# Chthi/Ofighters

Measured on AMD Instinct MI355X. Metric: arena-steps/sec (env.step+obs+policy fwd) at 4096 arenas, 1/2/4/8 MI355X, higher is better.
Workload: dtype f32; 1 GPU; 4096 arenas x 8 ships per GPU, random-bot actions + step + 2D obs rasterise (u8 maps) + bi-head policy forward for 8 ship(s)/arena, trunk shared per arena (BASELINE configs[3]); arenas_per_gpu=4096, ships=8, laser_cap=512, episode_ticks=200, parallelism=arena-sharded x1, RCCL all-reduce of episodic scores only, laser_overflow=0, last_episode_score_sum=70993, last_episode_arenas=4096

## Files before the change

### ofighters_amd/csrc/ofx_trunk.hip

```cpp
#include "ofx_trunk.h"
#include "ofx_diag.h"
#include "ofx_lowp.h"

typedef float f32x4 __attribute__((ext_vector_type(4)));
typedef float f32x2 __attribute__((ext_vector_type(2)));

template <int CIN, int COUT, int TH, int TW, int MODE, bool POOL, bool OUT_HWC>
__global__ __launch_bounds__(((TH / 2) * (TW / 2) + 63) / 64 * 64) void k_conv(ConvParams p) {
  constexpr int NT = (TH / 2) * (TW / 2);
  constexpr int NTB = (NT + 63) / 64 * 64;
  constexpr int TWP = TW + 2;
  __shared__ __align__(16) float tile[CIN][TH + 2][TWP];
  const int img = blockIdx.x / p.tiles, t = blockIdx.x - img * p.tiles;
  if (p.mask && !p.mask[img]) return;
  const int ty0 = (t / p.tiles_x) * TH, tx0 = (t % p.tiles_x) * TW;
  const int tid = threadIdx.x;
  const int H = p.H, W = p.W;

  constexpr int TOTAL = CIN * (TH + 2) * TWP;
  constexpr int SU = 8;
  for (int base = 0; base < TOTAL; base += NTB * SU) {
    float vals[SU];
#pragma unroll
    for (int u = 0; u < SU; u++) {
      const int e = base + u * NTB + tid;
      float v = 0.f;
      if (e < TOTAL) {
        const int c = e % TWP, r = (e / TWP) % (TH + 2), ci = e / (TWP * (TH + 2));
        const int gy = ty0 - 1 + r, gx = tx0 - 1 + c;
        if (gy >= 0 && gy < H && gx >= 0 && gx < W) {
          if (MODE == 0) {
            v = p.in[(((size_t)img * CIN + ci) * H + gy) * W + gx];
          } else if (MODE == 1) {
            const int cell = gy * W + gx;
            v = (float)((p.bits[ci][(size_t)img * p.bits_stride + (cell >> 5)] >> (cell & 31)) & 1u);
          }
        }
      }
      vals[u] = v;
    }
#pragma unroll
    for (int u = 0; u < SU; u++) {
      const int e = base + u * NTB + tid;
      if (e < TOTAL) (&tile[0][0][0])[e] = vals[u];
    }
  }
  __syncthreads();
  if (tid >= NT) return;
  const int tr = tid / (TW / 2), tc = tid - tr * (TW / 2);

  float acc[2][2][COUT];
#pragma unroll
  for (int i = 0; i < 2; i++)
#pragma unroll
    for (int j = 0; j < 2; j++)
#pragma unroll
      for (int co = 0; co < COUT; co++) acc[i][j][co] = 0.f;

#pragma unroll
  for (int ci = 0; ci < CIN; ci++) {
    float v[4][4];
#pragma unroll
    for (int r = 0; r < 4; r++) {
      const float2 lo = *reinterpret_cast<const float2 *>(&tile[ci][2 * tr + r][2 * tc]);
      const float2 hi = *reinterpret_cast<const float2 *>(&tile[ci][2 * tr + r][2 * tc + 2]);
      v[r][0] = lo.x; v[r][1] = lo.y; v[r][2] = hi.x; v[r][3] = hi.y;
    }
#pragma unroll
    for (int dy = 0; dy < 3; dy++)
#pragma unroll
      for (int dx = 0; dx < 3; dx++)
#pragma unroll
        for (int co = 0; co < COUT; co++) {
          const float wv = p.w[((dy * 3 + dx) * CIN + ci) * COUT + co];
#pragma unroll
          for (int i = 0; i < 2; i++)
#pragma unroll
            for (int j = 0; j < 2; j++) acc[i][j][co] = __builtin_fmaf(v[i + dy][j + dx], wv, acc[i][j][co]);
        }
  }

  const int oy = ty0 + 2 * tr, ox = tx0 + 2 * tc;
#pragma unroll
  for (int co = 0; co < COUT; co++) {
    const float bias = p.b[co];
// ... 218 lines not shown
  p.H = H; p.W = H;
  p.tiles_x = (H + 16 * NG - 1) / (16 * NG);
  p.tiles = p.tiles_x * (H / TH);
  if (p.tiles % TPW) { ofx_set_error("launch_convm: %d tiles per image not divisible by %d", p.tiles, TPW); return OFX_ERR_INVALID; }
  if (OUT_HWC && (H % 2 || H > 16 * NG)) { ofx_set_error("launch_convm: the 8-byte staging takes even rows of one tile width"); return OFX_ERR_INVALID; }
  p.images = images;
  hipLaunchKernelGGL((k_convm<CIN, TH, NG, MODE, OUT_HWC, TPW, LP>), dim3((unsigned)((images + 7) / 8 * 8 * (p.tiles / TPW))), dim3(256), 0,
                     h->stream, p);
  OFX_HIP(hipGetLastError());
  return OFX_OK;
}

template <int TH>
__global__ __launch_bounds__(256) void k_conv1_lut(ConvParams p, const float *lut) {
  constexpr int W = PS, H = PS, WR = 14;
  constexpr int W2 = W / 2, NPX = (TH / 2) * W2;
  __shared__ __align__(16) float slut[2 * 512 * 8];
  __shared__ unsigned rows[2][TH + 2][WR];
  const int tiles = H / TH;
  const int img = blockIdx.x / tiles, ty0 = (blockIdx.x - img * tiles) * TH;
  const int tid = threadIdx.x;
  for (int e = tid; e < 2 * 512 * 8 / 4; e += 256)
    reinterpret_cast<float4 *>(slut)[e] = reinterpret_cast<const float4 *>(lut)[e];
  for (int e = tid; e < 2 * (TH + 2) * WR; e += 256) {
    const int w = e % WR, r = (e / WR) % (TH + 2), ci = e / (WR * (TH + 2));
    const int gy = ty0 - 1 + r;
    unsigned out = 0u;
    if (gy >= 0 && gy < H) {
      const long long s0 = (long long)gy * W + 32 * w - 1;
      const unsigned *bits = p.bits[ci] + (size_t)img * p.bits_stride;
      const long long sw = s0 >> 5;
      const unsigned lo = (sw >= 0 && sw < (PS * PS) >> 5) ? bits[sw] : 0u;
      const unsigned hi = (sw + 1 < (PS * PS) >> 5) ? bits[sw + 1] : 0u;
      out = __funnelshift_r(lo, hi, (unsigned)(s0 & 31));
      const int xlo = 32 * w - 1;
      if (xlo < 0) out &= ~1u;
      const int over = xlo + 32 - W;
      if (over > 0) out = over >= 32 ? 0u : (out & (0xFFFFFFFFu >> over));
    }
    rows[ci][r][w] = out;
  }
  __syncthreads();
  float *const obase = p.out + ((size_t)img * 8 * (H / 2) + (ty0 >> 1)) * W2;
  constexpr int NQ = NPX / 4, QR = W2 / 4;
  for (int qd = tid; qd < NQ; qd += 256) {
    const int py = qd / QR, pq = qd - py * QR;
    const int x0 = 8 * pq;
    unsigned f[2][4];
#pragma unroll
    for (int ci = 0; ci < 2; ci++)
#pragma unroll
      for (int r = 0; r < 4; r++) {
        const unsigned *rw = &rows[ci][2 * py + r][x0 >> 5];
        f[ci][r] = __funnelshift_r(rw[0], rw[1], (unsigned)(x0 & 31)) & 1023u;
      }
    f32x4 m4[8];
#pragma unroll
    for (int j = 0; j < 4; j++) {
      f32x4 acc[4][2];
#pragma unroll
      for (int ci = 0; ci < 2; ci++)
#pragma unroll
        for (int q = 0; q < 4; q++) {
          const int dy = q >> 1, sh = 2 * j + (q & 1);
          const unsigned pat = ((f[ci][dy] >> sh) & 7u) | (((f[ci][dy + 1] >> sh) & 7u) << 3) | (((f[ci][dy + 2] >> sh) & 7u) << 6);
          const f32x4 *e = reinterpret_cast<const f32x4 *>(&slut[(ci * 512 + pat) * 8]);
          if (ci == 0) { acc[q][0] = e[0]; acc[q][1] = e[1]; }
          else { acc[q][0] += e[0]; acc[q][1] += e[1]; }
        }
#pragma unroll
      for (int co = 0; co < 8; co++) {
        float m;
        asm("v_max3_f32 %0, %1, %2, 0" : "=v"(m) : "v"(acc[0][co >> 2][co & 3]), "v"(acc[1][co >> 2][co & 3]));
        asm("v_max3_f32 %0, %1, %2, %3" : "=v"(m) : "v"(acc[2][co >> 2][co & 3]), "v"(acc[3][co >> 2][co & 3]), "v"(m));
        m4[co][j] = m;
      }
    }
    const unsigned off = (unsigned)(py * W2 + 4 * pq);
#pragma unroll
    for (int co = 0; co < 8; co++) *reinterpret_cast<f32x4 *>(obase + (size_t)co * (H / 2) * W2 + off) = m4[co];
  }
}

template <int WD, int RP, int LS, int PLS>
__device__ __forceinline__ void ts_gemm_phase(const float *abase, const float (&bw)[24], const f32x4 binit, int wv, int n16,
                                              int kq, int r, float *orow) {
  constexpr int NK = 24, NPX = RP * WD, NT = (NPX + 15) / 16;
  static_assert(WD % 4 == 0 && NT <= 64, "four M-tiles per wave at most");
  auto aof = [&](int j) -> int { return (4 * (j & 1)) * PLS + ((j >> 1) / 3) * LS + ((j >> 1) % 3); };
  auto finish = [&](const f32x4 d, int T) {
    float q0, q1;
    q0 = max_raw(max_raw(d[0], 0.f), d[1]);
    q1 = max_raw(max_raw(d[2], 0.f), d[3]);
    q0 = max_raw(q0, __builtin_bit_cast(float, __builtin_amdgcn_mov_dpp(__builtin_bit_cast(int, q0), 0xB1, 0xF, 0xF, true)));
    q1 = max_raw(q1, __builtin_bit_cast(float, __builtin_amdgcn_mov_dpp(__builtin_bit_cast(int, q1), 0xB1, 0xF, 0xF, true)));
    const int P = 16 * T + 4 * kq;
    const int rp = P / WD, x = P - rp * WD;
    if (r == 0 && P < NPX) *reinterpret_cast<float2 *>(orow + rp * (WD / 2) + (x >> 1)) = make_float2(q0, q1);
  };
  auto a_of_tile = [&](int T) -> const float * {
    const int P = min(16 * T + n16, NPX - 1);
    const int rp = P / WD, x = P - rp * WD;
    return abase + 2 * rp * LS + x;
  };
  if (wv + 48 < NT) {
    const float *a0 = a_of_tile(wv), *a1 = a_of_tile(wv + 16), *a2 = a_of_tile(wv + 32), *a3 = a_of_tile(wv + 48);
    f32x4 d0 = binit, d1 = binit, d2 = binit, d3 = binit;
#pragma unroll
    for (int j = 0; j < NK; j++) {
      d0 = __builtin_amdgcn_mfma_f32_16x16x4f32(a0[aof(j)], bw[j], d0, 0, 0, 0);
      d1 = __builtin_amdgcn_mfma_f32_16x16x4f32(a1[aof(j)], bw[j], d1, 0, 0, 0);
      d2 = __builtin_amdgcn_mfma_f32_16x16x4f32(a2[aof(j)], bw[j], d2, 0, 0, 0);
      d3 = __builtin_amdgcn_mfma_f32_16x16x4f32(a3[aof(j)], bw[j], d3, 0, 0, 0);
    }
    finish(d0, wv); finish(d1, wv + 16); finish(d2, wv + 32); finish(d3, wv + 48);
  } else {
#pragma unroll 1
    for (int T = wv; T < NT; T += 32) {
      const int T1 = T + 16;
      const float *a0 = a_of_tile(T);
      if (T1 < NT) {
        const float *a1 = a_of_tile(T1);
        f32x4 d0 = binit, d1 = binit;
#pragma unroll
        for (int j = 0; j < NK; j++) {
          d0 = __builtin_amdgcn_mfma_f32_16x16x4f32(a0[aof(j)], bw[j], d0, 0, 0, 0);
          d1 = __builtin_amdgcn_mfma_f32_16x16x4f32(a1[aof(j)], bw[j], d1, 0, 0, 0);
        }
        finish(d0, T);
        finish(d1, T1);
      } else {
        f32x4 d0 = binit;
#pragma unroll
        for (int j = 0; j < NK; j++) d0 = __builtin_amdgcn_mfma_f32_16x16x4f32(a0[aof(j)], bw[j], d0, 0, 0, 0);
        finish(d0, T);
      }
    }
  }
}

template <int WD, int RP, int LS, int PLS, int LP>
__device__ __forceinline__ void ts_gemm_phase_sparse(const float *abase, const float (&bw)[LP ? 1 : 24], const lp_x4 (&bwb)[6],
                                                     const f32x4 binit, int wv, int lane,
                                                     int n16, int kq, int r, float *orow, const unsigned *nz, float k2,
                                                     bool top, bool bottom, unsigned &n_exec, unsigned &n_all,
                                                     unsigned long long *dbg = nullptr) {
#if OFX_TRUNK_STAMPS
  unsigned long long g_last = __builtin_amdgcn_s_memtime();
#define TSG_STAMP(i) do { const unsigned long long t_ = __builtin_amdgcn_s_memtime(); dbg[i] += t_ - g_last; g_last = t_; } while (0)
#else
#define TSG_STAMP(i) do { } while (0)
#endif
  constexpr int NK = 24, NPX = RP * WD, NT = (NPX + 15) / 16;
  static_assert(WD % 4 == 0 && NT <= 64, "four M-tiles per wave at most");
  auto aof = [&](int j) -> int { return (4 * (j & 1)) * PLS + ((j >> 1) / 3) * LS + ((j >> 1) % 3); };
  int toff[6];
#pragma unroll
  for (int J = 0; J < 6; J++) {
    const int tap = 2 * J + (kq >> 1);
    toff[J] = (4 * (kq & 1) - kq) * PLS + (tap / 3) * LS + tap % 3;
  }
  auto mm1 = [&](const float *a0, f32x4 &d0) {
    if constexpr (LP != 0) {
#pragma unroll
      for (int J = 0; J < 6; J++) {
        const float *q0 = a0 + toff[J];
        d0 = lp_mfma16<LP ? LP : 1>(lp_pk4<LP ? LP : 1>(q0[0], q0[PLS], q0[2 * PLS], q0[3 * PLS]), bwb[J], d0);
      }
    } else {
#pragma unroll
      for (int j = 0; j < NK; j++) d0 = __builtin_amdgcn_mfma_f32_16x16x4f32(a0[aof(j)], bw[LP ? 0 : j], d0, 0, 0, 0);
    }
  };
  auto mm2 = [&](const float *a0, const float *a1, f32x4 &d0, f32x4 &d1) {
    if constexpr (LP != 0) {
#pragma unroll
      for (int J = 0; J < 6; J++) {
        const float *q0 = a0 + toff[J], *q1 = a1 + toff[J];
        const lp_x4 A0 = lp_pk4<LP ? LP : 1>(q0[0], q0[PLS], q0[2 * PLS], q0[3 * PLS]);
        const lp_x4 A1 = lp_pk4<LP ? LP : 1>(q1[0], q1[PLS], q1[2 * PLS], q1[3 * PLS]);
        d0 = lp_mfma16<LP ? LP : 1>(A0, bwb[J], d0);
        d1 = lp_mfma16<LP ? LP : 1>(A1, bwb[J], d1);
      }
    } else {
#pragma unroll
      for (int j = 0; j < NK; j++) {
        d0 = __builtin_amdgcn_mfma_f32_16x16x4f32(a0[aof(j)], bw[LP ? 0 : j], d0, 0, 0, 0);
        d1 = __builtin_amdgcn_mfma_f32_16x16x4f32(a1[aof(j)], bw[LP ? 0 : j], d1, 0, 0, 0);
      }
    }
  };
  auto finish = [&](const f32x4 d, int T) {
    float q0, q1;
    q0 = max_raw(max_raw(d[0], 0.f), d[1]);
    q1 = max_raw(max_raw(d[2], 0.f), d[3]);
    q0 = max_raw(q0, __builtin_bit_cast(float, __builtin_amdgcn_mov_dpp(__builtin_bit_cast(int, q0), 0xB1, 0xF, 0xF, true)));
    q1 = max_raw(q1, __builtin_bit_cast(float, __builtin_amdgcn_mov_dpp(__builtin_bit_cast(int, q1), 0xB1, 0xF, 0xF, true)));
    const int P = 16 * T + 4 * kq;
    const int rp = P / WD, x = P - rp * WD;
    if (r == 0 && P < NPX) *reinterpret_cast<float2 *>(orow + rp * (WD / 2) + (x >> 1)) = make_float2(q0, q1);
  };
  auto a_of_tile = [&](int T) -> const float * {
    const int P = min(16 * T + n16, NPX - 1);
    const int rp = P / WD, x = P - rp * WD;
    return abase + 2 * rp * LS + x;
  };
  unsigned long long run_mask;
  {
    const int T = lane, P = 16 * T, rp = P / WD, x = P - rp * WD;
    bool run = T < NT;
    if (run && !(x < 1 || x + 15 > WD - 2 || P + 15 >= NPX || (top && rp == 0) || (bottom && rp == RP - 1))) {
      const int w0 = (x - 1) >> 5, lo = (x - 1) & 31;
      const unsigned m0 = 0x3FFFFu << lo, m1 = lo + 18 > 32 ? (1u << (lo + 18 - 32)) - 1u : 0u;
      unsigned any = 0u;
#pragma unroll
      for (int rr = 0; rr < 4; rr++) {
        const unsigned *rw = nz + (2 * rp + rr) * 8 + w0;
        any |= (rw[0] & m0) | (rw[1] & m1);
      }
      run = any != 0u;
    }
    run_mask = __builtin_amdgcn_ballot_w64(run);
  }
  auto store_const = [&](int T) {
    const int P = 16 * T + 4 * kq, rp = P / WD, x = P - rp * WD;
    if (r == 0) *reinterpret_cast<float2 *>(orow + rp * (WD / 2) + (x >> 1)) = make_float2(k2, k2);
  };
  auto run1 = [&](int T0) {
    f32x4 d0 = binit;
    mm1(a_of_tile(T0), d0);
    finish(d0, T0);
  };
#pragma unroll 1
  for (int T = wv; T < NT; T += 16)
    if (!((run_mask >> T) & 1ull)) store_const(T);
  if (wv == 0) { n_all += (unsigned)NT; n_exec += (unsigned)__builtin_popcountll(run_mask); }
  TSG_STAMP(0);
  unsigned long long m = run_mask;
  for (int i = 0; i < wv && m; i++) m &= m - 1;
#pragma unroll 1
  while (m) {
    const int T0 = __builtin_ctzll(m);
    unsigned long long m2 = m;
    for (int i = 0; i < 16 && m2; i++) m2 &= m2 - 1;
    if (m2) {
      const int T1 = __builtin_ctzll(m2);
      f32x4 d0 = binit, d1 = binit;
      mm2(a_of_tile(T0), a_of_tile(T1), d0, d1);
      finish(d0, T0);
      finish(d1, T1);
      for (int i = 0; i < 16 && m2; i++) m2 &= m2 - 1;
    } else run1(T0);
    m = m2;
  }
  TSG_STAMP(2);
}

template <int WD, int RP, int LS, int PLS, int LP>
__device__ __forceinline__ void ts_gemm_phase_bf16(const float *abase, const lp_x4 (&bwb)[6], const f32x4 binit, int wv, int n16,
                                                   int kq, int r, float *orow) {
  constexpr int NPX = RP * WD, NT = (NPX + 15) / 16;
  static_assert(WD % 4 == 0 && NT <= 64, "four M-tiles per wave at most");
  int toff[6];
#pragma unroll
  for (int J = 0; J < 6; J++) {
    const int tap = 2 * J + (kq >> 1);
    toff[J] = (4 * (kq & 1) - kq) * PLS + (tap / 3) * LS + tap % 3;
  }
  auto finish = [&](const f32x4 d, int T) {
    float q0, q1;
    q0 = max_raw(max_raw(d[0], 0.f), d[1]);
    q1 = max_raw(max_raw(d[2], 0.f), d[3]);
    q0 = max_raw(q0, __builtin_bit_cast(float, __builtin_amdgcn_mov_dpp(__builtin_bit_cast(int, q0), 0xB1, 0xF, 0xF, true)));
    q1 = max_raw(q1, __builtin_bit_cast(float, __builtin_amdgcn_mov_dpp(__builtin_bit_cast(int, q1), 0xB1, 0xF, 0xF, true)));
    const int P = 16 * T + 4 * kq;
    const int rp = P / WD, x = P - rp * WD;
    if (r == 0 && P < NPX) *reinterpret_cast<float2 *>(orow + rp * (WD / 2) + (x >> 1)) = make_float2(q0, q1);
  };
  auto a_of_tile = [&](int T) -> const float * {
    const int P = min(16 * T + n16, NPX - 1);
    const int rp = P / WD, x = P - rp * WD;
    return abase + 2 * rp * LS + x;
  };
#pragma unroll 1
  for (int T = wv; T < NT; T += 32) {
    const int T1 = T + 16;
    const bool two = T1 < NT;
    const float *a0 = a_of_tile(T), *a1 = a_of_tile(two ? T1 : T);
    f32x4 d0 = binit, d1 = binit;
#pragma unroll
    for (int J = 0; J < 6; J++) {
      const float *q0 = a0 + toff[J], *q1 = a1 + toff[J];
      const lp_x4 A0 = lp_pk4<LP>(q0[0], q0[PLS], q0[2 * PLS], q0[3 * PLS]);
      const lp_x4 A1 = lp_pk4<LP>(q1[0], q1[PLS], q1[2 * PLS], q1[3 * PLS]);
      d0 = lp_mfma16<LP>(A0, bwb[J], d0);
      d1 = lp_mfma16<LP>(A1, bwb[J], d1);
    }
    finish(d0, T);
    if (two) finish(d1, T1);
  }
}

constexpr int F12_TH = 10, F12_LS = 216, F12_ROWS = F12_TH + 2;
constexpr int F12_PLS = (F12_ROWS * F12_LS + 63) / 64 * 64 + 16;
constexpr int F12_WR = 14, F12_BR = 2 * (F12_TH + 1) + 2;
constexpr int F12_THREADS = 1024;
static_assert(F12_PLS % 64 == 16 && F12_PLS % 4 == 0 && F12_LS % 4 == 0, "tile layout");
static_assert(2 * F12_BR * F12_WR <= F12_THREADS, "one staged word per thread");
static_assert((F12_TH + 1) * 100 <= 2 * F12_THREADS && F12_TH * 100 <= F12_THREADS, "pixel pairs per step");

template <int LP, bool SPARSE = false>
__global__ __launch_bounds__(F12_THREADS) void k_trunk12(ConvParams p, const float *lut) {
  constexpr bool BF16 = LP != 0;
  constexpr int W = PS, H = PS, H1 = PS / 2, H2 = PS / 4, LS = F12_LS, PLS = F12_PLS, NK = 24;
  __shared__ __align__(16) float slut[2 * 512 * 8];
  __shared__ __align__(16) float tile[8 * F12_PLS];
  __shared__ unsigned rows[2][2][F12_BR][F12_WR];
  __shared__ __align__(16) float halo[2][8][2][F12_LS];
  __shared__ unsigned nz[SPARSE ? 2 : 1][F12_ROWS][8];
  __shared__ __align__(16) float k1s[8], k2s[8];
  __shared__ float wbs[(SPARSE && !BF16) ? 24 * 64 : 1];
  unsigned n_exec = 0, n_all = 0, t_exec = 0, t_all = 0;
#if OFX_TRUNK_STAMPS
  unsigned long long st_a = 0, st_b = 0, st_last = __builtin_amdgcn_s_memtime(), st_begin = st_last, st_g[3] = {0, 0, 0};
#define T12_STAMP(acc) do { const unsigned long long t_ = __builtin_amdgcn_s_memtime(); acc += t_ - st_last; st_last = t_; } while (0)
#else
#define T12_STAMP(acc) do { } while (0)
#endif
  const int tid = threadIdx.x, lane = tid & 63;
  const int wv = __builtin_amdgcn_readfirstlane(tid >> 6);
  const int n16 = lane & 15, kq = lane >> 4, co = n16 >> 1, r = n16 & 1;

  auto bits_fetch = [&](int img, int pa, int pb) -> unsigned {
    const int nrows = 2 * (pb - pa) + 2;
    unsigned out = 0u;
    if (tid < 2 * nrows * F12_WR) {
      const int w = tid % F12_WR, rr = (tid / F12_WR) % nrows, ci = tid / (F12_WR * nrows);
      const int gy = 2 * pa - 1 + rr;
      if (gy >= 0 && gy < H) {
        const long long s0 = (long long)gy * W + 32 * w - 1;
        const unsigned *bits = p.bits[ci] + (size_t)img * p.bits_stride;
        const long long sw = s0 >> 5;
        const unsigned lo = (sw >= 0 && sw < (PS * PS) >> 5) ? bits[sw] : 0u;
        const unsigned hi = (sw + 1 < (PS * PS) >> 5) ? bits[sw + 1] : 0u;
        out = __funnelshift_r(lo, hi, (unsigned)(s0 & 31));
        const int xlo = 32 * w - 1;
        if (xlo < 0) out &= ~1u;
        const int over = xlo + 32 - W;
        if (over > 0) out = over >= 32 ? 0u : (out & (0xFFFFFFFFu >> over));
      }
    }
    return out;
  };
  auto bits_commit = [&](int buf, int pa, int pb, unsigned word) {
    const int nrows = 2 * (pb - pa) + 2;
    if (tid < 2 * nrows * F12_WR) {
      const int w = tid % F12_WR, rr = (tid / F12_WR) % nrows, ci = tid / (F12_WR * nrows);
      rows[buf][ci][rr][w] = word;
    }
  };

  for (int e = tid; e < 2 * 512 * 8 / 4; e += F12_THREADS)
    reinterpret_cast<f32x4 *>(slut)[e] = reinterpret_cast<const f32x4 *>(lut)[e];
  for (int e = tid; e < 8 * PLS / 4; e += F12_THREADS) reinterpret_cast<f32x4 *>(tile)[e] = f32x4{0.f, 0.f, 0.f, 0.f};
  for (int e = tid; e < 2 * 8 * 2 * LS / 4; e += F12_THREADS) reinterpret_cast<f32x4 *>(&halo[0][0][0][0])[e] = f32x4{0.f, 0.f, 0.f, 0.f};
  float bw[(BF16 || SPARSE) ? 1 : NK];
  lp_x4 bwb[6];
  if constexpr (BF16) ts_bw_lp<LP ? LP : 1>(p.wbm, n16, kq, bwb);
  else if constexpr (SPARSE) {
    for (int e = tid; e < NK * 64; e += F12_THREADS) wbs[e] = p.wbm[e];
  } else {
#pragma unroll
    for (int j = 0; j < NK; j++) bw[j] = p.wbm[j * 64 + lane];
  }
  const float bias = p.b[co];
  const f32x4 binit = {bias, bias, bias, bias};
  const float *abase = &tile[kq * PLS + 3];
  if constexpr (SPARSE) {
    __syncthreads();
    if (tid < 8) k1s[tid] = fmaxf(slut[tid] + slut[512 * 8 + tid], 0.f);
    for (int e = tid; e < 2 * F12_ROWS * 8; e += F12_THREADS) (&nz[0][0][0])[e] = 0u;
    __syncthreads();
    for (int e = tid; e < 8 * PLS; e += F12_THREADS) tile[e] = k1s[min(e / PLS, 7)];
    __syncthreads();
    if (wv == 0) {
      const float *a0 = abase + 2 * LS + 16 + n16;
      f32x4 d0 = binit;
      if constexpr (BF16) {
#pragma unroll
        for (int J = 0; J < 6; J++) {
          const int tap = 2 * J + (kq >> 1);
          const float *q0 = a0 + (4 * (kq & 1) - kq) * PLS + (tap / 3) * LS + tap % 3;
          d0 = lp_mfma16<LP ? LP : 1>(lp_pk4<LP ? LP : 1>(q0[0], q0[PLS], q0[2 * PLS], q0[3 * PLS]), bwb[J], d0);
        }
      } else {
        auto aof = [&](int j) -> int { return (4 * (j & 1)) * PLS + ((j >> 1) / 3) * LS + ((j >> 1) % 3); };
#pragma unroll
        for (int j = 0; j < NK; j++) d0 = __builtin_amdgcn_mfma_f32_16x16x4f32(a0[aof(j)], wbs[(BF16 ? 0 : j) * 64 + lane], d0, 0, 0, 0);
      }
      float q0 = max_raw(max_raw(d0[0], 0.f), d0[1]);
      q0 = max_raw(q0, __builtin_bit_cast(float, __builtin_amdgcn_mov_dpp(__builtin_bit_cast(int, q0), 0xB1, 0xF, 0xF, true)));
      if (r == 0 && kq == 0) k2s[co] = q0;
    }
    __syncthreads();
    for (int e = tid; e < 8 * PLS / 4; e += F12_THREADS) reinterpret_cast<f32x4 *>(tile)[e] = f32x4{0.f, 0.f, 0.f, 0.f};
  }
  bits_commit(0, 0, F12_TH + 1, bits_fetch((int)blockIdx.x, 0, F12_TH + 1));
  unsigned w_ahead = 0u;
  if constexpr (SPARSE) { if ((int)blockIdx.x < p.images) w_ahead = bits_fetch((int)blockIdx.x, F12_TH + 1, 2 * F12_TH + 1); }
  __syncthreads();
  const float k2 = SPARSE ? k2s[co] : 0.f;

#pragma unroll 1
  for (int img = (int)blockIdx.x; img < p.images; img += (int)gridDim.x)
#pragma unroll 1
  for (int step = 0; step < H1 / F12_TH; step++) {
    const int R0 = step * F12_TH;
    const int pa = step ? R0 + 1 : 0, pb = min(R0 + F12_TH + 1, H1);
    const int buf = step & 1;
    const bool last = step + 1 == H1 / F12_TH;
    const int nimg = last ? img + (int)gridDim.x : img;
    const bool more = nimg < p.images;
    const int na = last ? 0 : R0 + F12_TH + 1, nb = last ? F12_TH + 1 : min(R0 + 2 * F12_TH + 1, H1);
    unsigned nextw = 0u;
    T12_STAMP(st_b);
    if (step && pb - pa < F12_TH)
      for (int e = tid; e < 8 * LS; e += F12_THREADS) tile[(e / LS) * PLS + (F12_TH + 1) * LS + e % LS] = 0.f;
    if (!step)
      for (int e = tid; e < 8 * LS; e += F12_THREADS) tile[(e / LS) * PLS + e % LS] = 0.f;
    if (step && tid < 8 * 2 * (LS / 4)) {
      const int c4 = tid % (LS / 4), rr = (tid / (LS / 4)) & 1, ci = tid / (2 * (LS / 4));
      reinterpret_cast<f32x4 *>(&tile[ci * PLS + rr * LS])[c4] = reinterpret_cast<const f32x4 *>(&halo[buf][ci][rr][0])[c4];
    }
    if constexpr (SPARSE) {
      if (step && tid < 16) nz[buf][tid >> 3][tid & 7] = nz[buf ^ 1][F12_TH + (tid >> 3)][tid & 7];
    }
    for (int q = tid; q < (pb - pa) * 100; q += F12_THREADS) {
      const int py = q / 100, pp = q - py * 100;
      const int x0 = 4 * pp;
      unsigned f[2][4];
#pragma unroll
      for (int ci = 0; ci < 2; ci++)
#pragma unroll
        for (int rr = 0; rr < 4; rr++) {
          const unsigned *rw = &rows[buf][ci][2 * py + rr][x0 >> 5];
          f[ci][rr] = __funnelshift_r(rw[0], rw[1], (unsigned)(x0 & 31)) & 63u;
        }
      float m2[8][2];
      bool dense_pass = true;
      if constexpr (SPARSE) {
        const unsigned any = (f[0][0] | f[0][1] | f[0][2] | f[0][3]) | (f[1][0] | f[1][1] | f[1][2] | f[1][3]);
        dense_pass = __builtin_amdgcn_ballot_w64(any != 0u) != 0;
        t_all++;
        if (dense_pass) {
          t_exec++;
          if (any != 0u) atomicOr(&nz[buf][pa + py - (R0 - 1)][(2 * pp) >> 5], 3u << ((2 * pp) & 31));
        } else {
          const f32x4 ka = *reinterpret_cast<const f32x4 *>(&k1s[0]), kb = *reinterpret_cast<const f32x4 *>(&k1s[4]);
#pragma unroll
          for (int c = 0; c < 8; c++) m2[c][0] = m2[c][1] = c < 4 ? ka[c & 3] : kb[c & 3];
        }
      }
      if (dense_pass) {
#pragma unroll
      for (int j = 0; j < 2; j++) {
        f32x4 acc[4][2];
#pragma unroll
        for (int ci = 0; ci < 2; ci++)
#pragma unroll
          for (int qq = 0; qq < 4; qq++) {
            const int dy = qq >> 1, sh = 2 * j + (qq & 1);
            const unsigned pat = ((f[ci][dy] >> sh) & 7u) | (((f[ci][dy + 1] >> sh) & 7u) << 3) | (((f[ci][dy + 2] >> sh) & 7u) << 6);
            const f32x4 *e = reinterpret_cast<const f32x4 *>(&slut[(ci * 512 + pat) * 8]);
            if (ci == 0) { acc[qq][0] = e[0]; acc[qq][1] = e[1]; }
            else { acc[qq][0] += e[0]; acc[qq][1] += e[1]; }
          }
#pragma unroll
        for (int c = 0; c < 8; c++) {
          float m;
          asm("v_max3_f32 %0, %1, %2, 0" : "=v"(m) : "v"(acc[0][c >> 2][c & 3]), "v"(acc[1][c >> 2][c & 3]));
          asm("v_max3_f32 %0, %1, %2, %3" : "=v"(m) : "v"(acc[2][c >> 2][c & 3]), "v"(acc[3][c >> 2][c & 3]), "v"(m));
          m2[c][j] = m;
        }
      }
      }
      const int trow = pa + py - (R0 - 1);
      float *dst = &tile[trow * LS + 4 + 2 * pp];
#pragma unroll
      for (int c = 0; c < 8; c++) *reinterpret_cast<float2 *>(dst + c * PLS) = make_float2(m2[c][0], m2[c][1]);
      if (trow >= F12_TH) {
#pragma unroll
        for (int c = 0; c < 8; c++)
          *reinterpret_cast<float2 *>(&halo[buf ^ 1][c][trow - F12_TH][4 + 2 * pp]) = make_float2(m2[c][0], m2[c][1]);
      }
    }
    __syncthreads();

    T12_STAMP(st_a);
    if constexpr (!SPARSE) { if (more) nextw = bits_fetch(nimg, na, nb); }
    if constexpr (SPARSE) {
      if (more) bits_commit(buf ^ 1, na, nb, w_ahead);
      int i2 = nimg, s2 = last ? 0 : step + 1;
      if (++s2 == H1 / F12_TH) { s2 = 0; i2 += (int)gridDim.x; }
      const int r2 = s2 * F12_TH;
      w_ahead = i2 < p.images ? bits_fetch(i2, s2 ? r2 + 1 : 0, min(r2 + F12_TH + 1, H1)) : 0u;
    }

    if constexpr (SPARSE) {
      float bwl[BF16 ? 1 : NK];
      if constexpr (!BF16) {
        int zoff;
        asm volatile("s_mov_b32 %0, 0" : "=s"(zoff));
#pragma unroll
        for (int j = 0; j < NK; j++) bwl[j] = wbs[j * 64 + lane + zoff];
      }
      ts_gemm_phase_sparse<200, F12_TH / 2, F12_LS, F12_PLS, LP>(abase, bwl, bwb, binit, wv, lane, n16, kq, r,
                                                                  p.out + (((size_t)img * 8 + co) * H2 + (R0 >> 1)) * H2,
                                                                  &nz[buf][0][0], k2, step == 0, last, n_exec, n_all
#if OFX_TRUNK_STAMPS
                                                                  , st_g
#endif
                                                                  );
      for (int e = tid; e < F12_ROWS * 8; e += F12_THREADS) (&nz[buf ^ 1][0][0])[e] = 0u;
    } else if constexpr (BF16)
      ts_gemm_phase_bf16<200, F12_TH / 2, F12_LS, F12_PLS, LP ? LP : 1>(abase, bwb, binit, wv, n16, kq, r,
                                                            p.out + (((size_t)img * 8 + co) * H2 + (R0 >> 1)) * H2);
    else
      ts_gemm_phase<200, F12_TH / 2, F12_LS, F12_PLS>(abase, bw, binit, wv, n16, kq, r,
                                                       p.out + (((size_t)img * 8 + co) * H2 + (R0 >> 1)) * H2);
    if constexpr (!SPARSE) { if (more) bits_commit(buf ^ 1, na, nb, nextw); }
    __syncthreads();
  }
  if constexpr (SPARSE) {
#if OFX_TRUNK_STAMPS
    T12_STAMP(st_b);
    if (p.stat && tid == 0) {
      atomicAdd(&p.stat[0], st_a); atomicAdd(&p.stat[1], st_b);
      atomicAdd(&p.stat[2], st_g[0]); atomicAdd(&p.stat[3], st_g[2]);
    }
#else
    if (p.stat && lane == 0) {
      atomicAdd(&p.stat[0], (unsigned long long)n_exec); atomicAdd(&p.stat[1], (unsigned long long)n_all);
      atomicAdd(&p.stat[2], (unsigned long long)t_exec); atomicAdd(&p.stat[3], (unsigned long long)t_all);
    }
#endif
  }
}

constexpr int C3_W = 100, C3_TH = 20, C3_LS = 108, C3_ROWS = C3_TH + 2, C3_F4 = C3_LS / 4;
constexpr int C3_PLS = (C3_ROWS * C3_LS + 63) / 64 * 64 + 16;
constexpr int C3_PF4 = C3_ROWS * C3_F4, C3_NI = (C3_PF4 + 63) / 64;
static_assert(C3_PLS % 64 == 16 && C3_W % C3_TH == 0 && C3_W / 4 + 2 == C3_F4 && 64 * C3_NI * 4 <= C3_PLS + 64 * 4, "tile layout");
static_assert(2 * 8 * C3_PLS * 4 <= 160 * 1024, "two tiles in LDS");

template <int LP>
__global__ __launch_bounds__(F12_THREADS) void k_conv3_stream(ConvParams p, const float *zero16) {
  constexpr bool BF16 = LP != 0;
  constexpr int W = C3_W, H = C3_W, H2 = C3_W / 2, PLS = C3_PLS, NK = 24, STEPS = H / C3_TH;
  __shared__ __align__(16) float tiles[2][8 * C3_PLS];
  const int tid = threadIdx.x, lane = tid & 63;
  const int wv = __builtin_amdgcn_readfirstlane(tid >> 6);
  const int n16 = lane & 15, kq = lane >> 4, co = n16 >> 1, r = n16 & 1;

  auto stage = [&](int buf, int img, int R0) {
#pragma unroll 1
    for (int i = wv; i < 8 * C3_NI; i += F12_THREADS / 64) {
      const int ci = i / C3_NI, k = i - ci * C3_NI;
      const int q = 64 * k + lane;
      if (q < C3_PF4) {
        const int row = q / C3_F4, c4 = q - row * C3_F4, gy = R0 - 1 + row;
        const float *src = zero16;
        if (c4 >= 1 && c4 <= W / 4 && gy >= 0 && gy < H) src = p.in + (((size_t)img * 8 + ci) * H + gy) * W + 4 * (c4 - 1);
        __builtin_amdgcn_global_load_lds((const __attribute__((address_space(1))) void *)src,
                                         (__attribute__((address_space(3))) void *)&tiles[buf][ci * PLS + 256 * k], 16, 0, 0);
      }
    }
  };

  float bw[BF16 ? 1 : NK];
  lp_x4 bwb[6];
  if constexpr (BF16) ts_bw_lp<LP ? LP : 1>(p.wbm, n16, kq, bwb);
  else {
#pragma unroll
    for (int j = 0; j < NK; j++) bw[j] = p.wbm[j * 64 + lane];
  }
  const float bias = p.b[co];
  const f32x4 binit = {bias, bias, bias, bias};
  if ((int)blockIdx.x < p.images) stage(0, (int)blockIdx.x, 0);
  __builtin_amdgcn_s_waitcnt(0x0F70);
  __syncthreads();
  int buf = 0;
#pragma unroll 1
  for (int img = (int)blockIdx.x; img < p.images; img += (int)gridDim.x)
#pragma unroll 1
  for (int step = 0; step < STEPS; step++) {
    const int R0 = step * C3_TH;
    const bool last = step + 1 == STEPS;
    const int nimg = last ? img + (int)gridDim.x : img;
    if (nimg < p.images) stage(buf ^ 1, nimg, last ? 0 : R0 + C3_TH);
    if constexpr (BF16)
      ts_gemm_phase_bf16<W, C3_TH / 2, C3_LS, C3_PLS, LP ? LP : 1>(&tiles[buf][kq * PLS + 3], bwb, binit, wv, n16, kq, r,
                                                      p.out + (((size_t)img * 8 + co) * H2 + (R0 >> 1)) * H2);
    else
      ts_gemm_phase<W, C3_TH / 2, C3_LS, C3_PLS>(&tiles[buf][kq * PLS + 3], bw, binit, wv, n16, kq, r,
                                                 p.out + (((size_t)img * 8 + co) * H2 + (R0 >> 1)) * H2);
    __builtin_amdgcn_s_waitcnt(0x0F70);
    __syncthreads();
    buf ^= 1;
  }
}

bool ofx_trunk_fused(const ofx_handle *h, size_t N) {
  if (h->opt_trunk_plain) return false;
  return h->opt_trunk_fuse == 1 || (h->opt_trunk_fuse == 0 && N >= 4 * (size_t)h->n_cus);
}

template <int CIN, int COUT, int TH, int TW, int MODE, bool POOL, bool OUT_HWC>
static int launch_conv(ofx_handle *h, ConvParams p, int images, int H) {
  p.H = H; p.W = H;
  p.tiles_x = H / TW;
  p.tiles = p.tiles_x * (H / TH);
  constexpr int NTB = ((TH / 2) * (TW / 2) + 63) / 64 * 64;
  hipLaunchKernelGGL((k_conv<CIN, COUT, TH, TW, MODE, POOL, OUT_HWC>), dim3((unsigned)(images * p.tiles)), dim3(NTB), 0,
                     h->stream, p);
  OFX_HIP(hipGetLastError());
  return OFX_OK;
}

static int launch_conv1_lut(ofx_handle *h, ConvParams cp, const float *lut) {
  cp.H = PS; cp.W = PS;
  hipLaunchKernelGGL(k_conv1_lut<40>, dim3((unsigned)(cp.images * (PS / 40))), dim3(256), 0, h->stream, cp, lut);
  OFX_HIP(hipGetLastError());
  return OFX_OK;
}

int ofx_launch_conv1_lut(ofx_handle *h, const void *bits, int n, const float *lut, float *out) {
  ConvParams cp{};
  cp.bits[0] = reinterpret_cast<const unsigned *>(bits);
  cp.bits[1] = cp.bits[0] + (PS * PS) / 32;
  cp.bits_stride = 2 * (size_t)((PS * PS) / 32);
  cp.out = out; cp.images = n;
  return launch_conv1_lut(h, cp, lut);
}

static void trunk_layer(ConvParams &cp, const TrunkParams &p, int i, const float *in, float *out) {
  cp.in = in; cp.w = p.tw[i]; cp.b = p.tb[i]; cp.out = out;
  if (i > 0) cp.wbm = p.wbm[i - 1];
}

template <int LP>
static int trunk_streaming(ofx_handle *h, ConvParams cp, const TrunkParams &p) {
  const dim3 grid((unsigned)(p.images < h->n_cus ? p.images : h->n_cus));
  cp.w = p.tw[0]; cp.b = p.tb[1]; cp.out = p.p2; cp.wbm = p.wbm[0]; cp.stat = p.stat;
  if (p.sparse) hipLaunchKernelGGL((k_trunk12<LP, true>), grid, dim3(F12_THREADS), 0, h->stream, cp, p.lut1);
  else hipLaunchKernelGGL((k_trunk12<LP, false>), grid, dim3(F12_THREADS), 0, h->stream, cp, p.lut1);
  OFX_HIP(hipGetLastError());
  trunk_layer(cp, p, 2, p.p2, p.p3);
  hipLaunchKernelGGL(k_conv3_stream<LP>, grid, dim3(F12_THREADS), 0, h->stream, cp, p.zero16);
  OFX_HIP(hipGetLastError());
  trunk_layer(cp, p, 3, p.p3, p.p4);
  return launch_convm<8, 10, 4, 0, true, 1, LP>(h, cp, p.images, 50);
}

int ofx_launch_trunk(ofx_handle *h, const TrunkParams &p) {
  ConvParams cp{};
  cp.bits[0] = p.bits[0]; cp.bits[1] = p.bits[1]; cp.bits_stride = p.bits_stride; cp.images = p.images;
  const bool plain = h->opt_trunk_plain;
  if (ofx_trunk_fused(h, (size_t)p.images))
    return p.lowp == 1 ? trunk_streaming<1>(h, cp, p) : p.lowp == 2 ? trunk_streaming<2>(h, cp, p) : trunk_streaming<0>(h, cp, p);
  const int N = p.images;
  int rc;
  trunk_layer(cp, p, 0, nullptr, p.p1);
  if ((rc = plain ? launch_conv<2, 8, 10, 100, 1, true, false>(h, cp, N, 400) : launch_conv1_lut(h, cp, p.lut1))) return rc;
  trunk_layer(cp, p, 1, p.p1, p.p2);
  if ((rc = plain ? launch_conv<8, 8, 10, 100, 0, true, false>(h, cp, N, 200) : launch_convm<8, 2, 13, 0, false, 1>(h, cp, N, 200))) return rc;
  trunk_layer(cp, p, 2, p.p2, p.p3);
  if ((rc = plain ? launch_conv<8, 8, 10, 100, 0, true, false>(h, cp, N, 100) : launch_convm<8, 4, 7, 0, false, 1>(h, cp, N, 100))) return rc;
  trunk_layer(cp, p, 3, p.p3, p.p4);
  return plain ? launch_conv<8, 8, 10, 50, 0, true, true>(h, cp, N, 50) : launch_convm<8, 10, 4, 0, true, 1>(h, cp, N, 50);
}

extern "C" int ofx_policy_trunk_stats(ofx_handle *h, int64_t *counts_host) {
  if (!h || !counts_host) { ofx_set_error("ofx_policy_trunk_stats: null argument"); return OFX_ERR_INVALID; }
  for (int i = 0; i < 4; i++) counts_host[i] = 0;
  if (!h->trunk_stat) return OFX_OK;
  OFX_HIP(hipSetDevice(h->cfg.device));
  OFX_HIP(hipMemcpyAsync(counts_host, h->trunk_stat, 4 * sizeof(unsigned long long), hipMemcpyDeviceToHost, h->stream));
  OFX_HIP(hipMemsetAsync(h->trunk_stat, 0, 4 * sizeof(unsigned long long), h->stream));
  OFX_HIP(hipStreamSynchronize(h->stream));
  return OFX_OK;
}
```

Before: 219,300 arena-steps/s.

## Split bit-plane prefetch into issue/commit and overlap with trunk GEMM phases

```diff
diff --git a/ofighters_amd/csrc/ofx_trunk.hip b/ofighters_amd/csrc/ofx_trunk.hip
--- a/ofighters_amd/csrc/ofx_trunk.hip
+++ b/ofighters_amd/csrc/ofx_trunk.hip
@@ -1,6 +1,9 @@
 #include "ofx_trunk.h"
 #include "ofx_diag.h"
 #include "ofx_lowp.h"
+#if OFX_TRUNK_STAMPS
+#include <stdlib.h>
+#endif
 
 typedef float f32x4 __attribute__((ext_vector_type(4)));
 typedef float f32x2 __attribute__((ext_vector_type(2)));
@@ -385,9 +388,9 @@
   }
 }
 
-template <int WD, int RP, int LS, int PLS>
+template <int WD, int RP, int LS, int PLS, class Mid>
 __device__ __forceinline__ void ts_gemm_phase(const float *abase, const float (&bw)[24], const f32x4 binit, int wv, int n16,
-                                              int kq, int r, float *orow) {
+                                              int kq, int r, float *obase, unsigned ooff, Mid &&mid) {
   constexpr int NK = 24, NPX = RP * WD, NT = (NPX + 15) / 16;
   static_assert(WD % 4 == 0 && NT <= 64, "four M-tiles per wave at most");
   auto aof = [&](int j) -> int { return (4 * (j & 1)) * PLS + ((j >> 1) / 3) * LS + ((j >> 1) % 3); };
@@ -399,7 +402,7 @@
     q1 = max_raw(q1, __builtin_bit_cast(float, __builtin_amdgcn_mov_dpp(__builtin_bit_cast(int, q1), 0xB1, 0xF, 0xF, true)));
     const int P = 16 * T + 4 * kq;
     const int rp = P / WD, x = P - rp * WD;
-    if (r == 0 && P < NPX) *reinterpret_cast<float2 *>(orow + rp * (WD / 2) + (x >> 1)) = make_float2(q0, q1);
+    if (r == 0 && P < NPX) *reinterpret_cast<float2 *>(obase + (ooff + (unsigned)(rp * (WD / 2) + (x >> 1)))) = make_float2(q0, q1);
   };
   auto a_of_tile = [&](int T) -> const float * {
     const int P = min(16 * T + n16, NPX - 1);
@@ -416,10 +419,13 @@
       d2 = __builtin_amdgcn_mfma_f32_16x16x4f32(a2[aof(j)], bw[j], d2, 0, 0, 0);
       d3 = __builtin_amdgcn_mfma_f32_16x16x4f32(a3[aof(j)], bw[j], d3, 0, 0, 0);
     }
+    mid();
     finish(d0, wv); finish(d1, wv + 16); finish(d2, wv + 32); finish(d3, wv + 48);
   } else {
+    static_assert(NT >= 16, "every wave has an M-tile: the loop below runs at least once");
+    int T = wv;
 #pragma unroll 1
-    for (int T = wv; T < NT; T += 32) {
+    do {
       const int T1 = T + 16;
       const float *a0 = a_of_tile(T);
       if (T1 < NT) {
@@ -438,7 +444,8 @@
         for (int j = 0; j < NK; j++) d0 = __builtin_amdgcn_mfma_f32_16x16x4f32(a0[aof(j)], bw[j], d0, 0, 0, 0);
         finish(d0, T);
       }
-    }
+    } while ((T += 32) < NT);
+    mid();
   }
 }
 
@@ -559,9 +566,9 @@
   TSG_STAMP(2);
 }
 
-template <int WD, int RP, int LS, int PLS, int LP>
+template <int WD, int RP, int LS, int PLS, int LP, class Mid>
 __device__ __forceinline__ void ts_gemm_phase_bf16(const float *abase, const lp_x4 (&bwb)[6], const f32x4 binit, int wv, int n16,
-                                                   int kq, int r, float *orow) {
+                                                   int kq, int r, float *orow, Mid &&mid) {
   constexpr int NPX = RP * WD, NT = (NPX + 15) / 16;
   static_assert(WD % 4 == 0 && NT <= 64, "four M-tiles per wave at most");
   int toff[6];
@@ -602,14 +609,17 @@
     finish(d0, T);
     if (two) finish(d1, T1);
   }
+  mid();
 }
 
 constexpr int F12_TH = 10, F12_LS = 216, F12_ROWS = F12_TH + 2;
 constexpr int F12_PLS = (F12_ROWS * F12_LS + 63) / 64 * 64 + 16;
 constexpr int F12_WR = 14, F12_BR = 2 * (F12_TH + 1) + 2;
 constexpr int F12_THREADS = 1024;
+constexpr int F12_BW = 6;
+struct BitsRaw { unsigned lo, hi; };
+static_assert(F12_BR * F12_WR <= 64 * F12_BW && 2 * 64 * F12_BW <= F12_THREADS, "one staged word per thread, a channel per wave");
 static_assert(F12_PLS % 64 == 16 && F12_PLS % 4 == 0 && F12_LS % 4 == 0, "tile layout");
-static_assert(2 * F12_BR * F12_WR <= F12_THREADS, "one staged word per thread");
 static_assert((F12_TH + 1) * 100 <= 2 * F12_THREADS && F12_TH * 100 <= F12_THREADS, "pixel pairs per step");
 
 template <int LP, bool SPARSE = false>
@@ -623,43 +633,52 @@
   __shared__ unsigned nz[SPARSE ? 2 : 1][F12_ROWS][8];
   __shared__ __align__(16) float k1s[8], k2s[8];
   __shared__ float wbs[(SPARSE && !BF16) ? 24 * 64 : 1];
+  __shared__ lp_x4 wbl[(SPARSE && BF16) ? 6 * 64 : 1];
   unsigned n_exec = 0, n_all = 0, t_exec = 0, t_all = 0;
 #if OFX_TRUNK_STAMPS
   unsigned long long st_a = 0, st_b = 0, st_last = __builtin_amdgcn_s_memtime(), st_begin = st_last, st_g[3] = {0, 0, 0};
 #define T12_STAMP(acc) do { const unsigned long long t_ = __builtin_amdgcn_s_memtime(); acc += t_ - st_last; st_last = t_; } while (0)
+  unsigned long long st_d[7] = {0, 0, 0, 0, 0, 0, 0};
+  unsigned st_steps = 0;
+#define T12_SEC(i) do { if constexpr (!SPARSE) { __builtin_amdgcn_sched_barrier(0); T12_STAMP(st_d[i]); __builtin_amdgcn_sched_barrier(0); } } while (0)
 #else
 #define T12_STAMP(acc) do { } while (0)
+#define T12_SEC(i) do { } while (0)
 #endif
   const int tid = threadIdx.x, lane = tid & 63;
   const int wv = __builtin_amdgcn_readfirstlane(tid >> 6);
   const int n16 = lane & 15, kq = lane >> 4, co = n16 >> 1, r = n16 & 1;
 
-  auto bits_fetch = [&](int img, int pa, int pb) -> unsigned {
-    const int nrows = 2 * (pb - pa) + 2;
-    unsigned out = 0u;
-    if (tid < 2 * nrows * F12_WR) {
-      const int w = tid % F12_WR, rr = (tid / F12_WR) % nrows, ci = tid / (F12_WR * nrows);
+  const int bci = wv >= F12_BW ? 1 : 0;
+  const unsigned *const bplane = bci ? p.bits[1] : p.bits[0];
+  auto bits_thread = [&](int nrows, int &rr, int &w) -> bool {
+    const int bt = tid - bci * (64 * F12_BW);
+    rr = bt / F12_WR; w = bt - rr * F12_WR;
+    return wv < 2 * F12_BW && rr < nrows;
+  };
+  auto bits_issue = [&](int img, int pa, int nrows, BitsRaw &raw) {
+    int rr, w;
+    if (bits_thread(nrows, rr, w)) {
+      const int gy = min(max(2 * pa - 1 + rr, 0), H - 1);
+      const int sw = (gy * W + 32 * w - 1) >> 5;
+      const unsigned *bits = bplane + (size_t)img * p.bits_stride;
+      raw.lo = bits[(unsigned)min(max(sw, 0), ((PS * PS) >> 5) - 1)];
+      raw.hi = bits[(unsigned)min(max(sw + 1, 0), ((PS * PS) >> 5) - 1)];
+    }
+  };
+  auto bits_commit = [&](int buf, int pa, int nrows, const BitsRaw raw) {
+    int rr, w;
+    if (bits_thread(nrows, rr, w)) {
       const int gy = 2 * pa - 1 + rr;
-      if (gy >= 0 && gy < H) {
-        const long long s0 = (long long)gy * W + 32 * w - 1;
-        const unsigned *bits = p.bits[ci] + (size_t)img * p.bits_stride;
-        const long long sw = s0 >> 5;
-        const unsigned lo = (sw >= 0 && sw < (PS * PS) >> 5) ? bits[sw] : 0u;
-        const unsigned hi = (sw + 1 < (PS * PS) >> 5) ? bits[sw + 1] : 0u;
-        out = __funnelshift_r(lo, hi, (unsigned)(s0 & 31));
-        const int xlo = 32 * w - 1;
-        if (xlo < 0) out &= ~1u;
-        const int over = xlo + 32 - W;
-        if (over > 0) out = over >= 32 ? 0u : (out & (0xFFFFFFFFu >> over));
-      }
-    }
-    return out;
-  };
-  auto bits_commit = [&](int buf, int pa, int pb, unsigned word) {
-    const int nrows = 2 * (pb - pa) + 2;
-    if (tid < 2 * nrows * F12_WR) {
-      const int w = tid % F12_WR, rr = (tid / F12_WR) % nrows, ci = tid / (F12_WR * nrows);
-      rows[buf][ci][rr][w] = word;
+      const int s0 = gy * W + 32 * w - 1, sw = s0 >> 5;
+      const unsigned lo = (sw >= 0 && sw < (PS * PS) >> 5) ? raw.lo : 0u;
+      const unsigned hi = (sw + 1 < (PS * PS) >> 5) ? raw.hi : 0u;
+      unsigned out = __funnelshift_r(lo, hi, (unsigned)(s0 & 31));
+      const int xlo = 32 * w - 1;
+      if (xlo < 0) out &= ~1u;
+      const int over = xlo + 32 - W;
+      if (over > 0) out = over >= 32 ? 0u : (out & (0xFFFFFFFFu >> over));
+      rows[buf][bci][rr][w] = (gy >= 0 && gy < H) ? out : 0u;
     }
   };
 
@@ -707,10 +726,18 @@
     }
     __syncthreads();
     for (int e = tid; e < 8 * PLS / 4; e += F12_THREADS) reinterpret_cast<f32x4 *>(tile)[e] = f32x4{0.f, 0.f, 0.f, 0.f};
-  }
-  bits_commit(0, 0, F12_TH + 1, bits_fetch((int)blockIdx.x, 0, F12_TH + 1));
-  unsigned w_ahead = 0u;
-  if constexpr (SPARSE) { if ((int)blockIdx.x < p.images) w_ahead = bits_fetch((int)blockIdx.x, F12_TH + 1, 2 * F12_TH + 1); }
+    if constexpr (BF16) {
+      if (wv == 0) {
+#pragma unroll
+        for (int J = 0; J < 6; J++) wbl[J * 64 + lane] = bwb[J];
+      }
+    }
+  }
+  BitsRaw w_ahead = {0u, 0u};
+  BitsRaw nextw = {0u, 0u};
+  bits_issue((int)blockIdx.x, 0, F12_BR, nextw);
+  bits_commit(0, 0, F12_BR, nextw);
+  if constexpr (SPARSE) { if ((int)blockIdx.x < p.images) bits_issue((int)blockIdx.x, F12_TH + 1, 2 * F12_TH + 2, w_ahead); }
   __syncthreads();
   const float k2 = SPARSE ? k2s[co] : 0.f;
 
@@ -725,7 +752,7 @@
     const int nimg = last ? img + (int)gridDim.x : img;
     const bool more = nimg < p.images;
     const int na = last ? 0 : R0 + F12_TH + 1, nb = last ? F12_TH + 1 : min(R0 + 2 * F12_TH + 1, H1);
-    unsigned nextw = 0u;
+    const int nn = 2 * (nb - na) + 2;
     T12_STAMP(st_b);
     if (step && pb - pa < F12_TH)
       for (int e = tid; e < 8 * LS; e += F12_THREADS) tile[(e / LS) * PLS + (F12_TH + 1) * LS + e % LS] = 0.f;
@@ -733,11 +760,13 @@
       for (int e = tid; e < 8 * LS; e += F12_THREADS) tile[(e / LS) * PLS + e % LS] = 0.f;
     if (step && tid < 8 * 2 * (LS / 4)) {
       const int c4 = tid % (LS / 4), rr = (tid / (LS / 4)) & 1, ci = tid / (2 * (LS / 4));
-      reinterpret_cast<f32x4 *>(&tile[ci * PLS + rr * LS])[c4] = reinterpret_cast<const f32x4 *>(&halo[buf][ci][rr][0])[c4];
+      const int ht = __builtin_amdgcn_mov_dpp(tid, 0xE4, 0xF, 0xF, true);
+      reinterpret_cast<f32x4 *>(&tile[ci * PLS + rr * LS])[c4] = reinterpret_cast<const f32x4 *>(&halo[buf][0][0][0])[ht];
     }
     if constexpr (SPARSE) {
       if (step && tid < 16) nz[buf][tid >> 3][tid & 7] = nz[buf ^ 1][F12_TH + (tid >> 3)][tid & 7];
     }
+    T12_SEC(0);
     for (int q = tid; q < (pb - pa) * 100; q += F12_THREADS) {
       const int py = q / 100, pp = q - py * 100;
       const int x0 = 4 * pp;
@@ -797,28 +826,45 @@
           *reinterpret_cast<float2 *>(&halo[buf ^ 1][c][trow - F12_TH][4 + 2 * pp]) = make_float2(m2[c][0], m2[c][1]);
       }
     }
+    T12_SEC(1);
     __syncthreads();
+    T12_SEC(2);
 
     T12_STAMP(st_a);
-    if constexpr (!SPARSE) { if (more) nextw = bits_fetch(nimg, na, nb); }
+    if constexpr (!SPARSE) { if (more) bits_issue(nimg, na, nn, nextw); }
+    T12_SEC(3);
+    auto commit_next = [&]() {
+      if constexpr (!SPARSE) {
+        T12_SEC(4);
+        __builtin_amdgcn_s_waitcnt(0x0F70);
+        if (more) bits_commit(buf ^ 1, na, nn, nextw);
+        T12_SEC(5);
+      }
+    };
     if constexpr (SPARSE) {
-      if (more) bits_commit(buf ^ 1, na, nb, w_ahead);
+      if (more) bits_commit(buf ^ 1, na, nn, w_ahead);
       int i2 = nimg, s2 = last ? 0 : step + 1;
       if (++s2 == H1 / F12_TH) { s2 = 0; i2 += (int)gridDim.x; }
       const int r2 = s2 * F12_TH;
-      w_ahead = i2 < p.images ? bits_fetch(i2, s2 ? r2 + 1 : 0, min(r2 + F12_TH + 1, H1)) : 0u;
-    }
-
+      const int a2 = s2 ? r2 + 1 : 0;
+      if (i2 < p.images) bits_issue(i2, a2, 2 * (min(r2 + F12_TH + 1, H1) - a2) + 2, w_ahead);
+    }
+
+    float *const obase = p.out + ((size_t)img * 8 * H2 + (R0 >> 1)) * H2;
     if constexpr (SPARSE) {
       float bwl[BF16 ? 1 : NK];
+      lp_x4 bwh[6];
+      int zoff;
+      asm volatile("s_mov_b32 %0, 0" : "=s"(zoff));
       if constexpr (!BF16) {
-        int zoff;
-        asm volatile("s_mov_b32 %0, 0" : "=s"(zoff));
 #pragma unroll
         for (int j = 0; j < NK; j++) bwl[j] = wbs[j * 64 + lane + zoff];
-      }
-      ts_gemm_phase_sparse<200, F12_TH / 2, F12_LS, F12_PLS, LP>(abase, bwl, bwb, binit, wv, lane, n16, kq, r,
-                                                                  p.out + (((size_t)img * 8 + co) * H2 + (R0 >> 1)) * H2,
+      } else {
+#pragma unroll
+        for (int J = 0; J < 6; J++) bwh[J] = wbl[J * 64 + lane + zoff];
+      }
+      ts_gemm_phase_sparse<200, F12_TH / 2, F12_LS, F12_PLS, LP>(abase, bwl, bwh, binit, wv, lane, n16, kq, r,
+                                                                  obase + co * (H2 * H2),
                                                                   &nz[buf][0][0], k2, step == 0, last, n_exec, n_all
 #if OFX_TRUNK_STAMPS
                                                                   , st_g
@@ -827,13 +873,25 @@
       for (int e = tid; e < F12_ROWS * 8; e += F12_THREADS) (&nz[buf ^ 1][0][0])[e] = 0u;
     } else if constexpr (BF16)
       ts_gemm_phase_bf16<200, F12_TH / 2, F12_LS, F12_PLS, LP ? LP : 1>(abase, bwb, binit, wv, n16, kq, r,
-                                                            p.out + (((size_t)img * 8 + co) * H2 + (R0 >> 1)) * H2);
+                                                                        obase + co * (H2 * H2), commit_next);
     else
-      ts_gemm_phase<200, F12_TH / 2, F12_LS, F12_PLS>(abase, bw, binit, wv, n16, kq, r,
-                                                       p.out + (((size_t)img * 8 + co) * H2 + (R0 >> 1)) * H2);
-    if constexpr (!SPARSE) { if (more) bits_commit(buf ^ 1, na, nb, nextw); }
+      ts_gemm_phase<200, F12_TH / 2, F12_LS, F12_PLS>(abase, bw, binit, wv, n16, kq, r, obase, (unsigned)(co * (H2 * H2)), commit_next);
+    T12_SEC(4);
     __syncthreads();
-  }
+    T12_SEC(6);
+#if OFX_TRUNK_STAMPS
+    st_steps++;
+#endif
+  }
+#if OFX_TRUNK_STAMPS
+  if constexpr (!SPARSE) {
+    if (p.stat && lane == 0 && (wv == 0 || wv == 12)) {
+#pragma unroll
+      for (int i = 0; i < 7; i++) atomicAdd(&p.stat[(wv ? 8 : 0) + i], st_d[i]);
+      if (wv == 0) atomicAdd(&p.stat[7], (unsigned long long)st_steps);
+    }
+  }
+#endif
   if constexpr (SPARSE) {
 #if OFX_TRUNK_STAMPS
     T12_STAMP(st_b);
@@ -842,7 +900,7 @@
       atomicAdd(&p.stat[2], st_g[0]); atomicAdd(&p.stat[3], st_g[2]);
     }
 #else
-    if (p.stat && lane == 0) {
+    if (p.stat && __builtin_amdgcn_mbcnt_hi(~0u, __builtin_amdgcn_mbcnt_lo(~0u, 0u)) == 0) {
       atomicAdd(&p.stat[0], (unsigned long long)n_exec); atomicAdd(&p.stat[1], (unsigned long long)n_all);
       atomicAdd(&p.stat[2], (unsigned long long)t_exec); atomicAdd(&p.stat[3], (unsigned long long)t_all);
     }
@@ -889,10 +947,20 @@
   }
   const float bias = p.b[co];
   const f32x4 binit = {bias, bias, bias, bias};
+#if OFX_TRUNK_STAMPS
+  unsigned long long c_d[4] = {0, 0, 0, 0}, c_last = 0;
+  unsigned c_steps = 0;
+#define C3_SEC(i) do { __builtin_amdgcn_sched_barrier(0); const unsigned long long t_ = __builtin_amdgcn_s_memtime(); c_d[i] += t_ - c_last; c_last = t_; __builtin_amdgcn_sched_barrier(0); } while (0)
+#else
+#define C3_SEC(i) do { } while (0)
+#endif
   if ((int)blockIdx.x < p.images) stage(0, (int)blockIdx.x, 0);
   __builtin_amdgcn_s_waitcnt(0x0F70);
   __syncthreads();
   int buf = 0;
+#if OFX_TRUNK_STAMPS
+  c_last = __builtin_amdgcn_s_memtime();
+#endif
 #pragma unroll 1
   for (int img = (int)blockIdx.x; img < p.images; img += (int)gridDim.x)
 #pragma unroll 1
@@ -901,16 +969,35 @@
     const bool last = step + 1 == STEPS;
     const int nimg = last ? img + (int)gridDim.x : img;
     if (nimg < p.images) stage(buf ^ 1, nimg, last ? 0 : R0 + C3_TH);
+    C3_SEC(0);
     if constexpr (BF16)
       ts_gemm_phase_bf16<W, C3_TH / 2, C3_LS, C3_PLS, LP ? LP : 1>(&tiles[buf][kq * PLS + 3], bwb, binit, wv, n16, kq, r,
-                                                      p.out + (((size_t)img * 8 + co) * H2 + (R0 >> 1)) * H2);
+                                                      p.out + (((size_t)img * 8 + co) * H2 + (R0 >> 1)) * H2, [] {});
     else
       ts_gemm_phase<W, C3_TH / 2, C3_LS, C3_PLS>(&tiles[buf][kq * PLS + 3], bw, binit, wv, n16, kq, r,
-                                                 p.out + (((size_t)img * 8 + co) * H2 + (R0 >> 1)) * H2);
-    __builtin_amdgcn_s_waitcnt(0x0F70);
-    __syncthreads();
+                                                 p.out + ((size_t)img * 8 * H2 + (R0 >> 1)) * H2, (unsigned)(co * (H2 * H2)), [] {});
+    C3_SEC(1);
+    static_assert((C3_TH / 2 * C3_W + 15) / 16 == 63 && F12_THREADS / 64 == 16, "stores per wave: 4, the last wave 3");
+    if (wv + 48 < 63) __builtin_amdgcn_s_waitcnt(0x0F74);
+    else __builtin_amdgcn_s_waitcnt(0x0F73);
+    C3_SEC(2);
+    __atomic_signal_fence(__ATOMIC_SEQ_CST);
+    __builtin_amdgcn_s_waitcnt(0xC07F);
+    __builtin_amdgcn_s_barrier();
+    __atomic_signal_fence(__ATOMIC_SEQ_CST);
+    C3_SEC(3);
+#if OFX_TRUNK_STAMPS
+    c_steps++;
+#endif
     buf ^= 1;
   }
+#if OFX_TRUNK_STAMPS
+  if (p.stat && lane == 0 && (wv == 0 || wv == 12)) {
+#pragma unroll
+    for (int i = 0; i < 4; i++) atomicAdd(&p.stat[16 + (wv ? 4 : 0) + i], c_d[i]);
+    if (wv == 0) atomicAdd(&p.stat[24], (unsigned long long)c_steps);
+  }
+#endif
 }
 
 bool ofx_trunk_fused(const ofx_handle *h, size_t N) {
@@ -951,16 +1038,52 @@
   if (i > 0) cp.wbm = p.wbm[i - 1];
 }
 
+#if OFX_TRUNK_STAMPS
+static unsigned long long *g_stamp_buf = nullptr;
+static int g_stamp_calls = 0;
+static void trunk_stamps_print(ofx_handle *h) {
+  unsigned long long v[32];
+  if (hipStreamSynchronize(h->stream) != hipSuccess || hipMemcpy(v, g_stamp_buf, sizeof(v), hipMemcpyDeviceToHost) != hipSuccess) return;
+  static const char *const sec[7] = {"top", "table", "barrier A", "fetch", "M-tiles", "commit", "barrier B"};
+  static const char *const sec3[4] = {"load issue", "M-tiles", "wait", "barrier"};
+  const double n = v[7] ? (double)v[7] : 1.0, n3 = v[24] ? (double)v[24] : 1.0;
+  for (int w = 0; w < 2; w++) {
+    double sum = 0;
+    fprintf(stderr, "trunk stamps k_trunk12<0,false> wave %2d:", w ? 12 : 0);
+    for (int i = 0; i < 7; i++) { fprintf(stderr, " %s %.0f", sec[i], (double)v[8 * w + i] / n); sum += (double)v[8 * w + i] / n; }
+    fprintf(stderr, " | step %.0f (%.0f steps)\n", sum, n);
+  }
+  for (int w = 0; w < 2; w++) {
+    double sum = 0;
+    fprintf(stderr, "trunk stamps k_conv3_stream<0> wave %2d:", w ? 12 : 0);
+    for (int i = 0; i < 4; i++) { fprintf(stderr, " %s %.0f", sec3[i], (double)v[16 + 4 * w + i] / n3); sum += (double)v[16 + 4 * w + i] / n3; }
+    fprintf(stderr, " | step %.0f (%.0f steps)\n", sum, n3);
+  }
+}
+#endif
+
 template <int LP>
 static int trunk_streaming(ofx_handle *h, ConvParams cp, const TrunkParams &p) {
   const dim3 grid((unsigned)(p.images < h->n_cus ? p.images : h->n_cus));
   cp.w = p.tw[0]; cp.b = p.tb[1]; cp.out = p.p2; cp.wbm = p.wbm[0]; cp.stat = p.stat;
+#if OFX_TRUNK_STAMPS
+  bool stamped = false;
+  if (!p.sparse && LP == 0 && getenv("OFX_TRUNK_STAMPS") && ++g_stamp_calls == 20) {
+    if (!g_stamp_buf) OFX_HIP(hipMalloc((void **)&g_stamp_buf, 32 * sizeof(unsigned long long)));
+    OFX_HIP(hipMemsetAsync(g_stamp_buf, 0, 32 * sizeof(unsigned long long), h->stream));
+    cp.stat = g_stamp_buf;
+    stamped = true;
+  }
+#endif
   if (p.sparse) hipLaunchKernelGGL((k_trunk12<LP, true>), grid, dim3(F12_THREADS), 0, h->stream, cp, p.lut1);
   else hipLaunchKernelGGL((k_trunk12<LP, false>), grid, dim3(F12_THREADS), 0, h->stream, cp, p.lut1);
   OFX_HIP(hipGetLastError());
   trunk_layer(cp, p, 2, p.p2, p.p3);
   hipLaunchKernelGGL(k_conv3_stream<LP>, grid, dim3(F12_THREADS), 0, h->stream, cp, p.zero16);
   OFX_HIP(hipGetLastError());
+#if OFX_TRUNK_STAMPS
+  if (stamped) trunk_stamps_print(h);
+#endif
   trunk_layer(cp, p, 3, p.p3, p.p4);
   return launch_convm<8, 10, 4, 0, true, 1, LP>(h, cp, p.images, 50);
 }
```

Measured after the change: 221,200 arena-steps/s, median of 6. About the same (+0.9%).
